# Costava/heightmap-ray-marcher

Measured on AMD Instinct MI355X. Metric: ray-steps/s at 3840x2160, 4096^2 heightmap, higher is better.
Workload: dtype f64; 1 GPU; C3: 4096x4096 heightmap, 3840x2160, spherical hfov 180, step_dist 0.25, grid_width 1; ray_steps_per_frame=1197030646, rays_per_frame=8294400, hits_per_frame=1006074, parallelism=1 GPU, launches back to back on one stream

## Files before the change

### heightmap-ray-marcher_amd/__init__.py

```python
from .lib import (
    Camera, Config, HmrmError, Scene, SceneParams, Stats,
    Ray, RayHit, TraceParams, SegmentParams, Sun, Water, CellMapParams, CellRect, GeometryPlanes, LightPlanes, MAP_TOWARDS_POINT, MAP_WEIGHT, MAP_DIFFUSE, MAP_NO_SHADOWS, RAY_END, TRACE_INTERIOR, SHADE_DIFFUSE, SHADE_NO_SHADOWS, RAY_DTYPE, RAY_HIT_DTYPE, RAY_MISS, RAY_HIT, RAY_CAPPED, MAX_RAYS, as_rays,
    PERSPECTIVE, SPHERICAL, ORTHOGRAPHIC, NEAREST, BILINEAR, NEAREST_F32,
    HMRM_OK, HMRM_E_ARG, HMRM_E_IO, HMRM_E_IMAGE, HMRM_E_CONFIG, HMRM_E_DEVICE, HMRM_E_NOTERM,
    EXPORTED_SYMBOLS, LIB_PATH, NO_PROBE, AA_FACTORS, aa_flags,
    band_local_rows, debug_frame, degrees_to_rads, device_count, image_load, image_load_memory, kernel_src_sha,
    last_error, mip_layout, level_state, calibrate, pick_kernel, plan_order, rcp_error, orbit_camera, orbit_frame_owner, png_encode, record_orbit, record_orbit_multi, record_orbit_shaded, record_orbit_baked, record_orbit_water, LIGHT_U8, LIGHT_U16, WATER_OWN_COLOR, WATER_BAKED, Haze, HAZE_SKY, HAZE_LINEAR, HAZE_EXP, HAZE_EXP2, MAX_HAZE_ENTRIES, haze_table, MAX_VIEWS, camera_array, views_tables, shade_flags, map_flags, sky_directions, render_multi, set_device, write_png, write_ppm, write_pfm,
)
from . import synth
```

### heightmap-ray-marcher_amd/csrc/api_aux.cpp

```cpp
#include <algorithm>
#include <cstdlib>
#include <cstring>
#include <fstream>
#include <new>
#include <sstream>

#include "api_internal.hpp"
#include "config.hpp"
#include "host_pool.hpp"
#include "image_io.hpp"

struct hmrm_config {
	hmrm::Config cfg;
	std::string log_cache, warn_cache;
};

extern "C" {

int hmrm_debug_kernel_choice(const hmrm_scene *s) {
	if (!s) return fail(HMRM_E_ARG, "NULL argument");
	std::lock_guard<std::mutex> lk(const_cast<hmrm_scene *>(s)->mu);
	if (s->knobs.kernel != 0) return s->knobs.kernel;
	return s->choice.use_group ? (s->choice.with_records ? 3 : 1) : 0;
}
// ... 335 lines not shown
	if (cam->projection == HMRM_SPHERICAL) {
		double *cc = tables, *cs = tables + W, *rs = tables + 2 * W, *rc2 = tables + 2 * W + H;
		const int nc = cam->width, nr = cam->height;
		hmrm::parallel_ranges(nc + nr, 1024, [&](int b, int e) {
			if (b < nc) hmrm::fill_col_tables(hc, b, std::min(e, nc), cc, cs);
			if (e > nc) hmrm::fill_row_tables(hc, std::max(b, nc) - nc, e - nc, rs, rc2);
		});
	}
	double *o = out25;
	for (int i = 0; i < 3; ++i) *o++ = f.cam[i];
	for (int i = 0; i < 3; ++i) *o++ = f.upper_left[i];
	for (int i = 0; i < 3; ++i) *o++ = f.plane_right[i];
	for (int i = 0; i < 3; ++i) *o++ = f.plane_down[i];
	for (int i = 0; i < 3; ++i) *o++ = f.look[i];
	for (int i = 0; i < 3; ++i) *o++ = f.c0[i];
	for (int i = 0; i < 3; ++i) *o++ = f.c1[i];
	*o++ = f.nudge;
	*o++ = f.step_dist;
	*o++ = (double)f.grid_pow2;
	*o++ = f.inv_grid_width;
	return HMRM_OK;
}

int hmrm_debug_pick_kernel(int32_t forced, int32_t use_other, int32_t records_ok, int32_t scene_verdict, int32_t scene_with_records,
                           int32_t *with_records_after) {
	hmrm::KernelChoice choice;
	choice.use_group = scene_verdict != 0;
	choice.probed = choice.use_group;
	choice.with_records = scene_with_records != 0;
	const int k = hmrm::pick_fast_kernel(forced, use_other != 0, records_ok != 0, choice);
	if (with_records_after) *with_records_after = choice.with_records ? 1 : 0;
	return k;
}

int hmrm_debug_level_state(int32_t level, int32_t young, int32_t min_level, int32_t out[8]) {
	if (!out || level < 0 || level > hmrm::kMipLevels || min_level < 0 || min_level >= hmrm::kMipLevels)
		return fail(HMRM_E_ARG, "hmrm_debug_level_state: bad argument");
	const uint32_t b = (uint32_t)(hmrm::level_state_table() >> (8 * level)) & 0xffu;
	const int hs = (int)(b & 31u), back = (int)(b >> 5);
	const int lstep = hmrm::level_step(young ? 0 : -1);
	out[0] = hs;
	out[1] = back;
	out[2] = (back + 1) << hs;
	out[3] = lstep;
	out[4] = hmrm::level_coarser(level, lstep);
	out[5] = hmrm::level_finer(level, lstep, min_level);
// ... 31 lines not shown
```

### heightmap-ray-marcher_amd/csrc/api_internal.hpp

```cpp
#pragma once
#include <hip/hip_runtime_api.h>

#include <cstddef>
#include <cstdint>
#include <mutex>
#include <string>
#include <vector>

#include "../../include/hmrm.h"
#include "frame.hpp"
#include "launch_order.hpp"
#include "render.hpp"

#pragma GCC visibility push(hidden)
namespace hmrm {
extern thread_local std::string g_error;
int fail(int code, const std::string &msg);
}
using namespace hmrm;

#define HIP_TRY(expr)                                                                         \
	do {                                                                                      \
		hipError_t e_ = (expr);                                                               \
		if (e_ != hipSuccess)                                                                 \
			return fail(HMRM_E_DEVICE, std::string(#expr) + ": " + hipGetErrorString(e_));    \
	} while (0)

struct Knobs {
	int64_t step_cap = (int64_t)1 << 26;
	int kernel = 0;
	bool tile_order = true;
	int order_mode = 2;
	int diag_mode = 0;
	int min_level = -1;
	int finest_pause = -1;
	bool order_verbose = false;
	bool try_group = true;
	int min_plane_shift = 0;
	int seg_n = 0;
	int seg_b[3] = {0, 0, 0}, seg_c[3] = {0, 0, 0};
};

template <bool kPinned> struct Scratch {
	void *ptr = nullptr;
	size_t cap = 0;
	int reserve(size_t bytes) {
		if (bytes <= cap) return HMRM_OK;
		release();
		if (kPinned) HIP_TRY(hipHostMalloc(&ptr, bytes, hipHostMallocDefault));
		else HIP_TRY(hipMalloc(&ptr, bytes));
		cap = bytes;
		return HMRM_OK;
	}
	template <class T> T *as() const { return static_cast<T *>(ptr); }
	void release() {
		if (ptr) (void)(kPinned ? hipHostFree(ptr) : hipFree(ptr));
		ptr = nullptr;
		cap = 0;
	}
// ... 217 lines not shown
```

### heightmap-ray-marcher_amd/csrc/api_launch.cpp

```cpp
#include <algorithm>
#include <cstdio>
#include <cstring>

#include "api_internal.hpp"
#include "host_pool.hpp"

static_assert(sizeof(hmrm_sun) == 48, "hmrm_sun has padding");
static_assert(sizeof(hmrm_camera) == 3 * sizeof(int32_t) + 4 + 8 * sizeof(double), "hmrm_camera has padding");
static_assert(sizeof(hmrm_scene_params) == 6 * sizeof(double), "hmrm_scene_params has padding");
static_assert(HMRM_SHADE_DIFFUSE == hmrm::kShadeDiffuse && HMRM_SHADE_NO_SHADOWS == hmrm::kShadeNoShadows, "route_frame's flag bits");

namespace {

int ensure_meas(StreamCtx *c) {
	if (!c->d_meas) HIP_TRY(hipMalloc((void **)&c->d_meas, (size_t)kMaxMeasRows * hmrm::kMeasureStride * sizeof(unsigned long long)));
	if (!c->h_meas) {
		const size_t n = (size_t)kFrameSlots * 2 * kMaxMeasRows * sizeof(unsigned long long);
		HIP_TRY(hipHostMalloc((void **)&c->h_meas, n, hipHostMallocMapped));
		HIP_TRY(hipHostGetDevicePointer((void **)&c->h_meas_dev, c->h_meas, 0));
	}
	return HMRM_OK;
}

bool others_idle(hmrm_scene *s, StreamCtx *c) {
// ... 192 lines not shown

int prepare_frame(hmrm_scene *s, StreamCtx *c, const hmrm_camera *cam, hmrm::DevFrame *f, FrameSlot **slot_out) {
	const uint64_t thr_bits = *(const uint64_t *)&s->thr_max;
	FrameSlot *slot = nullptr;
	for (FrameSlot &sl : c->slots)
		if (sl.valid && memcmp(&sl.cam, cam, sizeof *cam) == 0 && memcmp(&sl.params, &s->params, sizeof s->params) == 0 &&
		    sl.thr_max_bits == thr_bits)
			slot = &sl;
	if (!slot) {
		slot = &c->slots[0];
		for (FrameSlot &sl : c->slots)
			if (!sl.valid || sl.stamp < slot->stamp) {
				slot = &sl;
				if (!sl.valid) break;
			}
		slot->valid = false;
		if (slot->cal.in_flight >= 0) HIP_TRY(hipEventSynchronize(slot->measured));
		slot->cal.reset();
		hmrm::HostCamera hc;
		to_host_camera(cam, &hc);
		double *cc = nullptr, *cs = nullptr, *rs = nullptr, *rc = nullptr;
		const size_t W = (size_t)cam->width, H = (size_t)cam->height;
		if (cam->projection == HMRM_SPHERICAL) {
			const size_t n = 2 * W + 2 * H;
			if (n > c->arena_n) {
				HIP_TRY(hipStreamSynchronize(c->stream));
				if (c->d_arena) (void)hipFree(c->d_arena);
				if (c->h_arena) (void)hipHostFree(c->h_arena);
				c->d_arena = c->h_arena = nullptr;
				c->arena_n = 0;
				for (FrameSlot &sl : c->slots) {
					if (sl.cam.projection == HMRM_SPHERICAL) sl.valid = false;
					sl.d_tables = sl.h_tables = nullptr;
				}
				const size_t per = (n + 31) & ~(size_t)31;
				HIP_TRY(hipMalloc((void **)&c->d_arena, per * kFrameSlots * sizeof(double)));
				HIP_TRY(hipHostMalloc((void **)&c->h_arena, per * kFrameSlots * sizeof(double), hipHostMallocMapped));
				HIP_TRY(hipHostGetDevicePointer((void **)&c->h_arena_dev, c->h_arena, 0));
				c->arena_n = per;
			}
			const size_t idx = (size_t)(slot - c->slots);
			slot->d_tables = c->d_arena + idx * c->arena_n;
			slot->h_tables = c->h_arena + idx * c->arena_n;
			if (!slot->uploaded) HIP_TRY(hipEventCreateWithFlags(&slot->uploaded, hipEventDisableTiming));
			else HIP_TRY(hipEventSynchronize(slot->uploaded));
			cc = slot->h_tables;
			cs = cc + W;
// ... 3 lines not shown
		hmrm::DevFrame &fr = slot->frame;
		hmrm::build_frame(hc, s->map_w, s->map_h, s->params.min_height, s->params.max_height, s->params.grid_width,
		                  &fr, nullptr, nullptr, nullptr, nullptr);
		if (cam->projection == HMRM_SPHERICAL) {
			const FrameSlot *row_donor = nullptr, *col_donor = nullptr;
			for (const FrameSlot &o : c->slots) {
				if (!o.valid || &o == slot || o.cam.projection != HMRM_SPHERICAL || !o.h_tables) continue;
				if (o.cam.width != cam->width || o.cam.hfov != cam->hfov) continue;
				if (!col_donor && o.cam.hang == cam->hang) col_donor = &o;
				if (!row_donor && o.cam.height == cam->height && o.cam.vang == cam->vang) row_donor = &o;
			}
			if (col_donor) memcpy(cc, col_donor->h_tables, 2 * W * sizeof(double));
			if (row_donor) memcpy(rs, row_donor->h_tables + 2 * (size_t)row_donor->cam.width, 2 * H * sizeof(double));
			const int nc = col_donor ? 0 : cam->width, nr = row_donor ? 0 : cam->height;
			if (nc + nr > 0)
				hmrm::parallel_ranges(nc + nr, 1024, [&](int b, int e) {
					if (b < nc) hmrm::fill_col_tables(hc, b, std::min(e, nc), cc, cs);
					if (e > nc) hmrm::fill_row_tables(hc, std::max(b, nc) - nc, e - nc, rs, rc);
				});
		}
		slot->row_cost.assign(((size_t)cam->height + kCostRows - 1) / kCostRows, 0.0f);
		hmrm::estimate_row_costs(fr, cc, cs, rs, rc, kCostRows, slot->row_cost.data());
		if (cam->projection == HMRM_SPHERICAL) {
			HIP_TRY(hmrm::launch_upload_tables(c->h_arena_dev + (slot->h_tables - c->h_arena), slot->d_tables, 2 * W + 2 * H, c->stream));
			HIP_TRY(hipEventRecord(slot->uploaded, c->stream));
			fr.col_cos_ha = slot->d_tables;
			fr.col_sin_ha = slot->d_tables + W;
			fr.row_sin_va = slot->d_tables + 2 * W;
			fr.row_cos_va = slot->d_tables + 2 * W + H;
		}
		if (cam->sampling == HMRM_BILINEAR) {
			const int rc2 = ensure_bilinear_pyramid(s);
			if (rc2 != HMRM_OK) return rc2;
		}
		finish_frame_record(s, cam->sampling, &fr);
		slot->cam = *cam;
		slot->params = s->params;
		slot->thr_max_bits = thr_bits;
		slot->valid = true;
		for (size_t k = s->settled.size(); k-- > 0;) {
			const hmrm_scene::SettledOrder &so = s->settled[k];
			if (memcmp(&so.cam, cam, sizeof *cam) != 0 || memcmp(&so.params, &s->params, sizeof s->params) != 0 || so.thr_max_bits != thr_bits) continue;
			slot->cal.adopt(so.order);
			break;
		}
	}
	slot->stamp = ++s->clock;
	*f = slot->frame;
	apply_scene_knobs(s, f);
	if (slot_out) *slot_out = slot;
	return HMRM_OK;
}

void finish_frame_record(const hmrm_scene *s, int sampling, hmrm::DevFrame *fr) {
	fr->thr_max = sampling == HMRM_BILINEAR ? s->thr_max_bil : s->thr_max;
	fr->min_level = 0;
	while (fr->min_level < hmrm::kMipLevels - 1 && hmrm::win_cells(fr->min_level) < fr->min_window)
		++fr->min_level;
	fr->mipbuf = s->d_mipbuf;
	fr->mipbuf_bil = s->d_mipbuf_bil;
	fr->mip_row = s->mip_row;
	fr->mip_plane_shift = s->mip_plane_shift;
}

void apply_scene_knobs(const hmrm_scene *s, hmrm::DevFrame *f) {
	f->step_cap = s->knobs.step_cap;
	f->diag_mode = s->knobs.diag_mode;
	if (s->knobs.min_level >= 0) f->min_level = s->knobs.min_level;
	if (s->knobs.finest_pause >= 0) f->finest_pause = s->knobs.finest_pause;
}

int pick_views_kernel(hmrm_scene *s, StreamCtx *c, int sampling, ViewsKernel *out) {
	const bool huge_side = s->map_w >= (1 << 24) || s->map_h >= (1 << 24);
	const hmrm::FrameRoute route = hmrm::route_frame(s->knobs.kernel, huge_side, sampling, false, true, false, 0u);
	if (route.refused) return fail(HMRM_E_ARG, "maps with a side of 2^24 cells or more support nearest sampling only");
	int rc = wait_for_measure_fence(s, c);
	if (rc) return rc;
	poll_shadow_probe(s);
	const bool use_group = s->knobs.kernel == 0 && s->knobs.try_group && s->choice.use_group;
	out->literal = route.literal;
	out->kind = (hmrm::FastKernel)hmrm::pick_fast_kernel(s->knobs.kernel, use_group, sampling == 0 && s->d_records, s->choice);
	if (!route.literal && out->kind == hmrm::kRecords && (rc = ensure_records(s))) return rc;
	return HMRM_OK;
}

int acquire_view_stage(StreamCtx *c, size_t doubles, uint64_t stamp, ViewStage **out) {
	ViewStage *pick = nullptr, *oldest = &c->view_stages[0];
	for (ViewStage &v : c->view_stages) {
		if (v.stamp < oldest->stamp) oldest = &v;
		bool free_now = !v.used;
// ... 123 lines not shown
```

### heightmap-ray-marcher_amd/csrc/api_scene.cpp

```cpp
#include <cstdio>
#include <cstdlib>
#include <cstring>
#include <new>
#include <vector>

#include "api_internal.hpp"

namespace hmrm {

thread_local std::string g_error;

int fail(int code, const std::string &msg) {
	g_error = msg;
	return code;
}

int set_error(int code, const char *msg) { return fail(code, msg ? msg : ""); }

}

namespace {

Knobs read_knobs() {
	Knobs k;
	if (const char *s = getenv("HMRM_STEP_CAP")) {
		const long long v = atoll(s);
		if (v > 0) k.step_cap = v > 0x7fffffffLL ? 0x7fffffffLL : (int64_t)v;
	}
	if (const char *s = getenv("HMRM_KERNEL")) k.kernel = strcmp(s, "simple") == 0 ? 2 : (strcmp(s, "group") == 0 ? 1 : (strcmp(s, "rec") == 0 ? 3 : 0));
	if (const char *s = getenv("HMRM_TILE_ORDER")) {
		k.tile_order = s[0] != '0';
		if (s[0] == '1' || s[0] == '2') k.order_mode = s[0] - '0';
	}
	if (const char *s = getenv("HMRM_DIAG_ITERS")) k.diag_mode = atoi(s);
	if (const char *s = getenv("HMRM_ORDER_VERBOSE")) k.order_verbose = s[0] == '1';
	if (const char *s = getenv("HMRM_TRY_GROUP")) k.try_group = s[0] != '0';
	if (const char *s = getenv("HMRM_TILE_SEGMENTS")) {
		int b = 0, c = 0, used = 0;
		while (k.seg_n < 3 && sscanf(s, "%d:%d%n", &b, &c, &used) == 2 && b >= 0 && c > 0) {
			k.seg_b[k.seg_n] = b;
			k.seg_c[k.seg_n] = c;
			++k.seg_n;
			s += used;
			if (*s != ',') break;
			++s;
		}
	}
	if (const char *s = getenv("HMRM_DEBUG_PLANE_SHIFT")) {
		const int v = atoi(s);
		if (v > 0 && v <= 28) k.min_plane_shift = v;
	}
	if (const char *s = getenv("HMRM_MIN_LEVEL"))
		if (s[0] >= '0' && s[0] < '0' + hmrm::kMipLevels) k.min_level = s[0] - '0';
	if (const char *s = getenv("HMRM_FINEST_PAUSE"))
		if (s[0] >= '0' && s[0] <= '9') k.finest_pause = s[0] - '0';
	return k;
}

void destroy_ctx(StreamCtx *c) {
// ... 424 lines not shown
```

### heightmap-ray-marcher_amd/csrc/camera.cpp

```cpp
#include "frame.hpp"

#include <cmath>
#include <cstring>

namespace hmrm {
namespace {

struct Vec3 {
	double x, y, z;
};
inline Vec3 operator+(Vec3 a, Vec3 b) { return Vec3{a.x + b.x, a.y + b.y, a.z + b.z}; }
inline Vec3 operator-(Vec3 a, Vec3 b) { return Vec3{a.x - b.x, a.y - b.y, a.z - b.z}; }
inline Vec3 operator-(Vec3 a) { return Vec3{-a.x, -a.y, -a.z}; }
inline Vec3 operator*(double s, Vec3 v) { return Vec3{s * v.x, s * v.y, s * v.z}; }
inline Vec3 cross(Vec3 a, Vec3 b) {
	return Vec3{a.y * b.z - b.y * a.z, a.z * b.x - b.z * a.x, a.x * b.y - b.x * a.y};
}
inline double dot(Vec3 a, Vec3 b) {
	const double px = a.x * b.x, py = a.y * b.y, pz = a.z * b.z;
	return px + py + pz;
}
inline Vec3 normalize(Vec3 v) {
	const double inv = 1.0 / std::sqrt(dot(v, v));
	return Vec3{v.x * inv, v.y * inv, v.z * inv};
// ... 10 lines not shown
}

void fill_col_tables(const HostCamera &cam, int32_t begin, int32_t end, double *col_cos_ha, double *col_sin_ha) {
	const double hfov = cam.hfov;
	const double ul_hang = cam.hang + (hfov / 2.0);
	for (int32_t px = begin; px < end; ++px) {
		const double w = (double)px / (cam.width - 1);
		const double ha = ul_hang - w * hfov;
		col_cos_ha[px] = std::cos(ha);
		col_sin_ha[px] = std::sin(ha);
	}
}

void fill_row_tables(const HostCamera &cam, int32_t begin, int32_t end, double *row_sin_va, double *row_cos_va) {
	const double aspect = (double)cam.width / cam.height;
	const double vfov = cam.hfov / aspect;
	const double ul_vang = cam.vang - (vfov / 2.0);
	for (int32_t py = begin; py < end; ++py) {
		const double h = (double)py / (cam.height - 1);
		const double va = ul_vang + h * vfov;
		row_sin_va[py] = std::sin(va);
		row_cos_va[py] = std::cos(va);
	}
}

void fill_scene_fields(int32_t map_w, int32_t map_h, double min_height, double max_height, double grid_width,
                       double step_dist, DevFrame *f) {
	f->map_w = map_w;
	f->map_h = map_h;

	f->c0[0] = 0.0;
	f->c0[1] = 0.0;
	f->c0[2] = min_height;
	f->c1[0] = f->c0[0] + map_w * grid_width;
	f->c1[1] = f->c0[1] - map_h * grid_width;
	f->c1[2] = max_height;

	f->grid_width = grid_width;
	f->nudge = grid_width * 0.01;
	f->step_dist = step_dist;

	int e = 0;
	const double m = std::frexp(grid_width, &e);
	f->grid_pow2 = (std::isfinite(grid_width) && m == 0.5 && e > -1000 && e < 1000) ? 1 : 0;
	f->inv_grid_width = 1.0 / grid_width;
	f->grid_mode = grid_width == 1.0 ? 0 : (f->grid_pow2 ? 1 : 2);
// ... 74 lines not shown
```

### heightmap-ray-marcher_amd/csrc/frame.hpp

```cpp
#pragma once
#include <stdint.h>

namespace hmrm {

struct DevFrame {
	int32_t screen_w, screen_h;
	int32_t projection;
	int32_t map_w, map_h;
	uint8_t bg[4];
	double cam[3];
	double upper_left[3], plane_right[3], plane_down[3];
	double look[3];
	const double *col_cos_ha, *col_sin_ha;
	const double *row_sin_va, *row_cos_va;
	double c0[3], c1[3];
	double grid_width;
	double nudge;
	double step_dist;
	double inv_grid_width;
	int32_t grid_pow2;
	int32_t grid_mode;
	double thr_max;
	int64_t step_cap;
	const float *mipbuf;
// ... 93 lines not shown
	uint32_t spare1[2];
};
static_assert(sizeof(WindowRecord) == 32, "two 16-byte loads");
static_assert(kRecLevel >= kDenseFrom && kLevelStep == 1, "the record level's windows: 16 cells, every 4");
#if defined(__HIPCC__)
__host__ __device__
#endif
inline int rec_row(int map_w) { return (map_w + 3) >> 2; }

struct RowMap {
	int32_t row_begin;
	int32_t local_rows;
	int32_t band_rows;
	int32_t band_index, band_count;
	int32_t seg_first[3];
	int32_t seg_delta[4];
	unsigned long long *measure;
};
constexpr int kMeasureStride = 33;
constexpr int kOrderSegs = 4;

static_assert(sizeof(DevFrame) == 352,"DevFrame must not grow");

struct BatchRay { double pos[3], dir[3]; };
struct BatchHit {
	double point[3];
	double entry_d;
	uint32_t steps;
	int32_t cell_x, cell_y;
	uint8_t rgba[4];
	uint32_t status;
	uint32_t reserved;
};
static_assert(sizeof(BatchRay) == 48 && sizeof(BatchHit) == 56, "hmrm_ray / hmrm_ray_hit");
struct RayBatch {
	const BatchRay *rays;
	BatchHit *hits;
	int64_t n;
};
constexpr int kBatchW = 8;

struct SegRules {
	const uint32_t *max_steps;
	uint32_t limit;
	uint32_t interior;
};
// ... 61 lines not shown
	uint32_t flags;
};
constexpr uint32_t kHazeSky = 2u;
constexpr int kMaxHazeEntries = 4096;

struct HostCamera {
	int32_t width, height, projection;
	uint8_t bg_r, bg_g, bg_b, sampling;
	double hfov, hang, vang, pos[3], ortho_width, step_dist;
};

void build_frame(const HostCamera &cam, int32_t map_w, int32_t map_h,
                 double min_height, double max_height, double grid_width,
                 DevFrame *out,
                 double *col_cos_ha, double *col_sin_ha,
                 double *row_sin_va, double *row_cos_va);

void fill_scene_fields(int32_t map_w, int32_t map_h, double min_height, double max_height, double grid_width,
                       double step_dist, DevFrame *out);

void fill_col_tables(const HostCamera &cam, int32_t begin, int32_t end, double *col_cos_ha, double *col_sin_ha);
void fill_row_tables(const HostCamera &cam, int32_t begin, int32_t end, double *row_sin_va, double *row_cos_va);

void estimate_row_costs(const DevFrame &f, const double *col_cos_ha, const double *col_sin_ha,
                        const double *row_sin_va, const double *row_cos_va, int rows_per_sample, float *out);

}
```

### heightmap-ray-marcher_amd/csrc/march_frame.hpp

```cpp
#pragma once
#include "march.hpp"

namespace hmrm {

#ifdef HMRM_TIMELINE
__device__ __forceinline__ void timeline_wave_done(unsigned long long t0);
static void timeline_before_launch(dim3 grid, int tiles_y, const RowMap &rows);
#endif

template <int PROJ, bool STATS, int GWM, int LEAP, int SAMP, bool AA>
__global__ __launch_bounds__(kBlockThreads, HMRM_MIN_WAVES) HMRM_OCCUPANCY_ATTR void k_render_fast(const DevFrame f, const RowMap rows,
                                                     const double *__restrict__ thr,
                                                     const uint32_t *__restrict__ cmap,
                                                     uint32_t *__restrict__ out, int64_t out_stride_px,
                                                     int tiles_y, StatsOut st) {
#ifdef HMRM_TIMELINE
	const unsigned long long tl_t0 = __builtin_amdgcn_s_memrealtime();
#endif
	unsigned long long wave_t0 = 0;
	if (!STATS && rows.measure) wave_t0 = __builtin_amdgcn_s_memrealtime();
	const int tile_y = render_wave_tile<Family<FramesOf<STATS, AA>, PROJ, GWM, LEAP, SAMP>>(
	    f, rows, thr, cmap, out, out_stride_px, tiles_y, st, (int)blockIdx.x, blockIdx.z * 32768u + blockIdx.y, (int)(threadIdx.x >> 6),
	    (int)(threadIdx.x & 63));
	if (!STATS && rows.measure && tile_y >= 0 && (threadIdx.x & 63) == 0) {
		const unsigned long long took = __builtin_amdgcn_s_memrealtime() - wave_t0;
		unsigned long long *rec = rows.measure + (size_t)tile_y * kMeasureStride;
		if (blockIdx.x == 0 && threadIdx.x == 0) rec[0] = wave_t0;
		atomicMax(&rec[1 + (blockIdx.x & 31u)], took);
	}
#ifdef HMRM_TIMELINE
	if (!STATS) timeline_wave_done(tl_t0);
#endif
}

template <bool AA>
static hipError_t launch_fast(const DevFrame &f, const RowMap &rows, const double *d_thr_f64, const float *d_thr32,
                              const uint32_t *d_cmap, uint32_t *d_out, int64_t out_stride_px,
                              unsigned long long *d_counters, uint32_t *d_steps, double *d_entry, bool stats,
                              FastKernel kernel, const WindowRecord *d_records, hipStream_t stream) {
	DevFrame fr = f;
	const double *d_thr = nullptr;
	if (const hipError_t e = select_tables(&fr, kernel, d_thr_f64, d_thr32, d_records, &d_thr); e != hipSuccess) return e;
	const LaunchGrid g = tile_grid(f, rows);
	if (g.tiles_y == 0) return g.err;
	const StatsOut st{d_counters, d_steps, d_entry};
#ifdef HMRM_TIMELINE
	if (!stats) timeline_before_launch(g.grid, g.tiles_y, rows);
#endif
	auto launch = [&](auto instrumented) {
		dispatch_march(f.projection, f.grid_mode, kernel, f.sampling, [&](auto proj, auto gwm, auto leap, auto samp) {
			hipLaunchKernelGGL((k_render_fast<proj(), decltype(instrumented)::value, gwm(), leap(), samp(), AA>), g.grid,
			                   dim3(kBlockThreads), 0, stream, fr, rows, d_thr, d_cmap, d_out, out_stride_px, g.tiles_y, st);
		});
	};
	if (stats) launch(std::true_type{});
	else launch(std::false_type{});
	return hipGetLastError();
}

}
```

### heightmap-ray-marcher_amd/lib.py

```python
from __future__ import annotations

import ctypes as C
import os

import numpy as np

_HERE = os.path.dirname(os.path.abspath(__file__))
LIB_PATH = os.path.join(_HERE, "libhmrm.so")

HMRM_OK = 0
HMRM_E_ARG, HMRM_E_IO, HMRM_E_IMAGE, HMRM_E_CONFIG, HMRM_E_DEVICE, HMRM_E_NOTERM = -1, -2, -3, -4, -5, -6
PERSPECTIVE, SPHERICAL, ORTHOGRAPHIC = 1, 2, 3
NEAREST, BILINEAR, NEAREST_F32 = 0, 1, 2
_PROJ_NAMES = {"perspective": 1, "spherical": 2, "orthographic": 3}


NO_PROBE = 1
AA_FACTORS = (1, 2, 4, 8)


def aa_flags(n: int) -> int:
    return (int(n) & 15) << 8


# ... 296 lines not shown
        "hmrm_config_get_haze": (None, [vp, C.POINTER(Haze), vp]),
        "hmrm_config_haze_law": (i32, [vp]),
        "hmrm_config_haze_density": (C.c_double, [vp]),
        "hmrm_config_haze_far": (C.c_double, [vp]),
        "hmrm_render_shaded": (C.c_int, [vp, C.POINTER(Camera), C.POINTER(Sun), C.c_uint32, vp, C.c_size_t]),
        "hmrm_render_shaded_aa": (C.c_int, [vp, C.POINTER(Camera), C.POINTER(Sun), C.c_uint32, i32, vp, C.c_size_t]),
        "hmrm_render_shaded_begin": (C.c_int, [vp, C.POINTER(Camera), C.POINTER(Sun), C.c_uint32, C.c_uint32, C.POINTER(i32)]),
        "hmrm_render_shaded_device_begin": (C.c_int, [vp, C.POINTER(Camera), C.POINTER(Sun), C.c_uint32, vp, C.c_size_t, C.c_uint32,
                                                      C.POINTER(i32)]),
        "hmrm_scene_set_light": (C.c_int, [vp, vp, C.c_size_t, i32, C.c_uint32]),
        "hmrm_scene_set_light_device": (C.c_int, [vp, vp, C.c_size_t, i32, C.c_uint32, vp]),
        "hmrm_scene_bake_light": (C.c_int, [vp, C.POINTER(CellMapParams), dp, i32]),
        "hmrm_scene_clear_light": (C.c_int, [vp]),
        "hmrm_scene_light": (C.c_int, [vp, vp, C.c_size_t, C.POINTER(C.c_uint32)]),
        "hmrm_render_baked": (C.c_int, [vp, C.POINTER(Camera), C.c_uint32, i32, vp, C.c_size_t]),
        "hmrm_render_baked_begin": (C.c_int, [vp, C.POINTER(Camera), C.c_uint32, C.c_uint32, C.POINTER(i32)]),
        "hmrm_render_baked_device_begin": (C.c_int, [vp, C.POINTER(Camera), C.c_uint32, vp, C.c_size_t, C.c_uint32, C.POINTER(i32)]),
        "hmrm_record_orbit_baked": (C.c_int, [C.POINTER(vp), i32, C.POINTER(Camera), C.c_double, C.c_double, C.c_double,
                                              C.c_double, i32, C.c_char_p, C.c_longlong, i32, i32, C.c_uint32, C.c_uint32]),
        "hmrm_config_baked_light": (i32, [vp]),
        "hmrm_pick": (C.c_int, [vp, C.POINTER(Camera), i32, i32, C.POINTER(RayHit)]),
        "hmrm_debug_ray": (C.c_int, [vp, C.POINTER(Camera), i32, i32, dp, dp, dp]),
        "hmrm_debug_frame": (C.c_int, [C.POINTER(Camera), C.POINTER(SceneParams), i32, i32, vp, vp]),
        "hmrm_debug_plan_order": (C.c_int, [vp, i32, i32, C.POINTER(i32), C.POINTER(i32), vp]),
        "hmrm_debug_rcp_error": (C.c_int, [i32, C.c_uint64, C.c_uint64, i32, i32, dp, C.POINTER(C.c_uint64)]),
        "hmrm_last_kernel_ms": (C.c_double, []),
        "hmrm_bench_kernel_ms": (C.c_double, [vp, C.POINTER(Camera), i32]),
        "hmrm_orbit_camera": (None, [C.POINTER(Camera), C.c_double, C.c_double, C.c_double, C.c_double, i32, i32,
                                     C.POINTER(Camera)]),
        "hmrm_record_orbit": (C.c_int, [vp, C.POINTER(Camera), C.c_double, C.c_double, C.c_double, C.c_double, i32,
                                        C.c_char_p, C.c_longlong, i32, i32]),
        "hmrm_config_record_mode": (i32, [vp]),
        "hmrm_config_devices": (i32, [vp]),
        "hmrm_config_antialias": (i32, [vp]),
        "hmrm_config_interior": (i32, [vp]),
        "hmrm_config_shadows": (i32, [vp]),
        "hmrm_config_shading": (i32, [vp]),
        "hmrm_config_sky_light": (i32, [vp]),
        "hmrm_config_sun_scope": (i32, [vp]),
        "hmrm_config_sun_map_path": (C.c_char_p, [vp]),
        "hmrm_config_sun_map_lift": (C.c_double, [vp]),
        "hmrm_config_sky_map_path": (C.c_char_p, [vp]),
        "hmrm_config_sky_map_rings": (None, [vp, C.POINTER(i32), C.POINTER(i32)]),
        "hmrm_config_range_map_path": (C.c_char_p, [vp]),
        "hmrm_config_get_sun": (None, [vp, C.POINTER(Sun)]),
        "hmrm_record_orbit_multi": (C.c_int, [C.POINTER(vp), i32, C.POINTER(Camera), C.c_double, C.c_double, C.c_double,
# ... 86 lines not shown


def _check(rc: int, allow=()):
    if rc != HMRM_OK and rc not in allow:
        raise HmrmError(rc, last_error())
    return rc


def _ptr(a: np.ndarray):
    return a.ctypes.data_as(C.c_void_p)


def device_count() -> int:
    n = lib.hmrm_device_count()
    if n < 0:
        raise HmrmError(n, last_error())
    return n


def set_device(i: int):
    _check(lib.hmrm_set_device(int(i)))


_ENV_KNOBS = ("HMRM_KERNEL", "HMRM_STEP_CAP", "HMRM_TILE_ORDER", "HMRM_DIAG_ITERS", "HMRM_MIN_LEVEL", "HMRM_FINEST_PAUSE", "HMRM_TILE_SEGMENTS", "HMRM_ORDER_VERBOSE", "HMRM_TRY_GROUP")


def shade_flags(diffuse=True, shadows=True) -> int:
    return (SHADE_DIFFUSE if diffuse else 0) | (0 if shadows else SHADE_NO_SHADOWS)


def map_flags(point=False, weight=False, diffuse=False, shadows=True) -> int:
    return ((MAP_TOWARDS_POINT if point else 0) | (MAP_WEIGHT if weight else 0) | (MAP_DIFFUSE if diffuse else 0)
            | (0 if shadows else MAP_NO_SHADOWS))


def sky_directions(rings: int, per_ring: int) -> np.ndarray:
    n = int(rings) * int(per_ring)
    out = np.zeros((max(min(n, 256), 1), 3), dtype=np.float64)
    rc = lib.hmrm_sky_directions(int(rings), int(per_ring), out.ctypes.data_as(C.POINTER(C.c_double)))
    if rc < 0:
        raise HmrmError(rc, last_error())
    return out[:rc]


def _as_rect(rect):
    if rect is None or isinstance(rect, CellRect):
        return rect
# ... 457 lines not shown

    def bench_kernel_ms(self, cam: Camera, iters: int) -> float:
        self._sync_env()
        ms = lib.hmrm_bench_kernel_ms(self._h, C.byref(cam), int(iters))
        if ms < 0:
            raise HmrmError(HMRM_E_DEVICE, last_error())
        return ms


def debug_frame(cam: Camera, params: SceneParams, map_w: int, map_h: int):
    out = np.empty(25, dtype=np.float64)
    tables = np.empty(2 * cam.width + 2 * cam.height, dtype=np.float64)
    _check(lib.hmrm_debug_frame(C.byref(cam), C.byref(params), map_w, map_h, _ptr(out), _ptr(tables)))
    W, H = cam.width, cam.height
    rec = {"cam": out[0:3], "upper_left": out[3:6], "plane_right": out[6:9], "plane_down": out[9:12],
           "look": out[12:15], "c0": out[15:18], "c1": out[18:21], "nudge": out[21], "step_dist": out[22],
           "grid_pow2": int(out[23]), "inv_grid_width": out[24]}
    if cam.projection == SPHERICAL:
        rec.update(col_cos_ha=tables[0:W], col_sin_ha=tables[W:2 * W],
                   row_sin_va=tables[2 * W:2 * W + H], row_cos_va=tables[2 * W + H:])
    return rec


def mip_layout(map_w: int, map_h: int):
    row, shift, levels = C.c_int32(), C.c_int32(), C.c_int32()
    rc = lib.hmrm_debug_mip_layout(int(map_w), int(map_h), C.byref(row), C.byref(shift), C.byref(levels))
    if rc < 0:
        raise HmrmError(rc, last_error())
    return row.value, shift.value, levels.value, bool(rc)


def level_state(level: int, young: bool, min_level: int):
    out = (C.c_int32 * 8)()
    rc = lib.hmrm_debug_level_state(int(level), int(bool(young)), int(min_level), out)
    if rc < 0:
        raise HmrmError(rc, last_error())
    keys = ("stride_shift", "back", "cells", "lstep", "coarser", "finer", "at_finest", "byte")
    return dict(zip(keys, (int(v) for v in out))), int(rc)


def pick_kernel(forced=0, use_other=False, records_ok=True, verdict=False, verdict_with_records=False):
    after = C.c_int32()
    k = lib.hmrm_debug_pick_kernel(int(forced), int(use_other), int(records_ok), int(verdict), int(verdict_with_records), C.byref(after))
    return int(k), bool(after.value)


# ... 340 lines not shown
```

### include/hmrm.h

```cpp
#ifndef HMRM_H
#define HMRM_H

#include <stddef.h>
#include <stdint.h>

#ifdef __cplusplus
extern "C" {
#endif

#define HMRM_ABI_VERSION 1

enum {
	HMRM_OK          =  0,
	HMRM_E_ARG       = -1,
	HMRM_E_IO        = -2,
	HMRM_E_IMAGE     = -3,
	HMRM_E_CONFIG    = -4,
	HMRM_E_DEVICE    = -5,
	HMRM_E_NOTERM    = -6
};

enum {
	HMRM_PERSPECTIVE  = 1,
	HMRM_SPHERICAL    = 2,
// ... 269 lines not shown
	uint8_t  reserved[5];
} hmrm_haze;
int hmrm_render_haze(const hmrm_scene *scene, const hmrm_camera *cam, const hmrm_haze *haze, const uint8_t *table, int32_t factor,
                     uint8_t *rgba, size_t stride_bytes);
int hmrm_render_haze_device(const hmrm_scene *scene, const hmrm_camera *cam, const hmrm_haze *haze, const void *d_table,
                            int32_t factor, void *d_rgba, size_t stride_bytes, void *hip_stream);
int hmrm_haze_table(int32_t law, double density, int32_t n, uint8_t *out);

#define HMRM_MAX_VIEWS 65536
#define HMRM_MAX_VIEWS_STAGING (256u << 20)
int hmrm_render_views(const hmrm_scene *scene, const hmrm_camera *cams, int32_t n, uint32_t flags,
                      uint8_t *rgba, size_t stride_bytes, size_t view_stride_bytes);
int hmrm_render_views_device(const hmrm_scene *scene, const hmrm_camera *cams, int32_t n, uint32_t flags,
                             void *d_rgba, size_t stride_bytes, size_t view_stride_bytes, void *hip_stream);
int hmrm_debug_views_tables(const hmrm_camera *cams, int32_t n, int32_t *out_col_index, int32_t *out_row_index);

int hmrm_pick(const hmrm_scene *scene, const hmrm_camera *cam, int32_t px, int32_t py, hmrm_ray_hit *hit);

int hmrm_debug_ray(const hmrm_scene *scene, const hmrm_camera *cam,
                   int32_t px, int32_t py, double pos[3], double dir[3], double *entry_d);

int hmrm_debug_frame(const hmrm_camera *cam, const hmrm_scene_params *params,
                     int32_t map_w, int32_t map_h, double *out25, double *tables);

int hmrm_debug_plan_order(const uint64_t *records, int32_t tile_rows, int32_t rot, int32_t pieces_begin[3],
                          int32_t pieces_count[3], int32_t *tile_row_of_grid_row);

int hmrm_debug_calibrate(const uint64_t *records, int32_t launches, int32_t tile_rows, int32_t rot, int32_t may_probe,
                         int32_t scene_already_probed, const uint8_t *can_measure, int32_t *trial_used, int32_t *measured,
                         int32_t *group_kernel, int32_t *n_trials, int32_t *best, int32_t *scene_use_group,
                         int32_t *settled_at_launch);

int hmrm_debug_level_state(int32_t level, int32_t young, int32_t min_level, int32_t out[8]);

int hmrm_debug_rcp_error(int32_t mode, uint64_t count, uint64_t seed, int32_t exp_lo, int32_t exp_hi,
                         double *max_rel_err, uint64_t *hist64);

int hmrm_debug_mip_layout(int32_t map_w, int32_t map_h, int32_t *mip_row, int32_t *plane_shift, int32_t *levels);

int hmrm_debug_kernel_choice(const hmrm_scene *scene);

int hmrm_debug_read_records(const hmrm_scene *scene, void *records_out, double *thr_out);

int hmrm_debug_pick_kernel(int32_t forced, int32_t use_other, int32_t records_ok, int32_t scene_verdict, int32_t scene_with_records,
                           int32_t *with_records_after);

// ... 91 lines not shown
```

Before: 12540 billion ray-steps/s.

## Skip marching for 8x8 sky tiles proven to miss the heightmap box

On the host, per-row and per-column sign classes of the spherical ray directions are built, along with a per-row sky colour, and uploaded alongside the trig tables. In the fast kernel, a wave whose 8x8 tile is proven to point away from the heightmap bounding box writes the precomputed sky colour and skips the ray-march. This removes setup and marching cost for rays that can never hit terrain. It adds host table construction, a larger upload, a per-wave classification check, and an env knob to turn it off. It is gated off for stats, AA, and row maps not aligned to 8 rows.

```diff
diff --git a/heightmap-ray-marcher_amd/__init__.py b/heightmap-ray-marcher_amd/__init__.py
--- a/heightmap-ray-marcher_amd/__init__.py
+++ b/heightmap-ray-marcher_amd/__init__.py
@@ -4,7 +4,7 @@
     PERSPECTIVE, SPHERICAL, ORTHOGRAPHIC, NEAREST, BILINEAR, NEAREST_F32,
     HMRM_OK, HMRM_E_ARG, HMRM_E_IO, HMRM_E_IMAGE, HMRM_E_CONFIG, HMRM_E_DEVICE, HMRM_E_NOTERM,
     EXPORTED_SYMBOLS, LIB_PATH, NO_PROBE, AA_FACTORS, aa_flags,
-    band_local_rows, debug_frame, degrees_to_rads, device_count, image_load, image_load_memory, kernel_src_sha,
+    band_local_rows, debug_frame, debug_sky_tables, degrees_to_rads, device_count, image_load, image_load_memory, kernel_src_sha,
     last_error, mip_layout, level_state, calibrate, pick_kernel, plan_order, rcp_error, orbit_camera, orbit_frame_owner, png_encode, record_orbit, record_orbit_multi, record_orbit_shaded, record_orbit_baked, record_orbit_water, LIGHT_U8, LIGHT_U16, WATER_OWN_COLOR, WATER_BAKED, Haze, HAZE_SKY, HAZE_LINEAR, HAZE_EXP, HAZE_EXP2, MAX_HAZE_ENTRIES, haze_table, MAX_VIEWS, camera_array, views_tables, shade_flags, map_flags, sky_directions, render_multi, set_device, write_png, write_ppm, write_pfm,
 )
 from . import synth
diff --git a/heightmap-ray-marcher_amd/csrc/api_aux.cpp b/heightmap-ray-marcher_amd/csrc/api_aux.cpp
--- a/heightmap-ray-marcher_amd/csrc/api_aux.cpp
+++ b/heightmap-ray-marcher_amd/csrc/api_aux.cpp
@@ -381,6 +381,33 @@
 	return HMRM_OK;
 }
 
+int hmrm_debug_sky_tables(const hmrm_camera *cam, const hmrm_scene_params *params, int32_t map_w, int32_t map_h,
+                          uint32_t *row_miss_rgba, uint32_t *row_class, uint32_t *col_class, uint32_t box_side[3],
+                          int32_t box_side_known[3], uint8_t *proven) {
+	int rc = check_camera(cam);
+	if (rc) return rc;
+	if (!params || !row_miss_rgba || !row_class || !col_class) return fail(HMRM_E_ARG, "NULL argument");
+	if (cam->projection != HMRM_SPHERICAL) return fail(HMRM_E_ARG, "hmrm_debug_sky_tables: spherical cameras only");
+	hmrm::HostCamera hc;
+	to_host_camera(cam, &hc);
+	const size_t W = (size_t)cam->width, H = (size_t)cam->height;
+	std::vector<double> tables(2 * W + 2 * H);
+	double *cc = tables.data(), *cs = cc + W, *rs = cs + W, *rc2 = rs + H;
+	hmrm::DevFrame f;
+	hmrm::build_frame(hc, map_w, map_h, params->min_height, params->max_height, params->grid_width, &f, cc, cs, rs, rc2);
+	hmrm::build_sky_tables(f, cc, cs, rs, rc2, row_miss_rgba, row_class, col_class);
+	for (int i = 0; i < 3; ++i) {
+		if (box_side) box_side[i] = f.box_side[i];
+		if (box_side_known) box_side_known[i] = f.box_side_known[i];
+	}
+	if (proven) {
+		const int gx = hmrm::sky_groups(cam->width), gy = hmrm::sky_groups(cam->height);
+		for (int y = 0; y < gy; ++y)
+			for (int x = 0; x < gx; ++x) proven[(size_t)y * gx + x] = hmrm::sky_tile_proven(f, row_class[y], col_class[x]) ? 1 : 0;
+	}
+	return HMRM_OK;
+}
+
 int hmrm_debug_pick_kernel(int32_t forced, int32_t use_other, int32_t records_ok, int32_t scene_verdict, int32_t scene_with_records,
                            int32_t *with_records_after) {
 	hmrm::KernelChoice choice;
diff --git a/heightmap-ray-marcher_amd/csrc/api_internal.hpp b/heightmap-ray-marcher_amd/csrc/api_internal.hpp
--- a/heightmap-ray-marcher_amd/csrc/api_internal.hpp
+++ b/heightmap-ray-marcher_amd/csrc/api_internal.hpp
@@ -35,6 +35,7 @@
 	int min_level = -1;
 	int finest_pause = -1;
 	bool order_verbose = false;
+	bool sky_tiles = true;
 	bool try_group = true;
 	int min_plane_shift = 0;
 	int seg_n = 0;
diff --git a/heightmap-ray-marcher_amd/csrc/api_launch.cpp b/heightmap-ray-marcher_amd/csrc/api_launch.cpp
--- a/heightmap-ray-marcher_amd/csrc/api_launch.cpp
+++ b/heightmap-ray-marcher_amd/csrc/api_launch.cpp
@@ -238,7 +238,7 @@
 		double *cc = nullptr, *cs = nullptr, *rs = nullptr, *rc = nullptr;
 		const size_t W = (size_t)cam->width, H = (size_t)cam->height;
 		if (cam->projection == HMRM_SPHERICAL) {
-			const size_t n = 2 * W + 2 * H;
+			const size_t n = 2 * W + 2 * H + hmrm::sky_table_doubles(cam->width, cam->height);
 			if (n > c->arena_n) {
 				HIP_TRY(hipStreamSynchronize(c->stream));
 				if (c->d_arena) (void)hipFree(c->d_arena);
@@ -288,7 +288,12 @@
 		slot->row_cost.assign(((size_t)cam->height + kCostRows - 1) / kCostRows, 0.0f);
 		hmrm::estimate_row_costs(fr, cc, cs, rs, rc, kCostRows, slot->row_cost.data());
 		if (cam->projection == HMRM_SPHERICAL) {
-			HIP_TRY(hmrm::launch_upload_tables(c->h_arena_dev + (slot->h_tables - c->h_arena), slot->d_tables, 2 * W + 2 * H, c->stream));
+			const size_t sky_doubles = hmrm::sky_table_doubles(cam->width, cam->height);
+			uint32_t *sky = reinterpret_cast<uint32_t *>(rc + H);
+			sky[2 * sky_doubles - 1] = 0u;
+			hmrm::build_sky_tables(fr, cc, cs, rs, rc, sky, sky + H, sky + H + hmrm::sky_groups(cam->height));
+			fr.diag_mode = hmrm::kSkyTilesUsable;
+			HIP_TRY(hmrm::launch_upload_tables(c->h_arena_dev + (slot->h_tables - c->h_arena), slot->d_tables, 2 * W + 2 * H + sky_doubles, c->stream));
 			HIP_TRY(hipEventRecord(slot->uploaded, c->stream));
 			fr.col_cos_ha = slot->d_tables;
 			fr.col_sin_ha = slot->d_tables + W;
@@ -331,7 +336,7 @@
 
 void apply_scene_knobs(const hmrm_scene *s, hmrm::DevFrame *f) {
 	f->step_cap = s->knobs.step_cap;
-	f->diag_mode = s->knobs.diag_mode;
+	f->diag_mode = (s->knobs.diag_mode & ~hmrm::kSkyTilesUsable) | (s->knobs.sky_tiles ? (f->diag_mode & hmrm::kSkyTilesUsable) : 0);
 	if (s->knobs.min_level >= 0) f->min_level = s->knobs.min_level;
 	if (s->knobs.finest_pause >= 0) f->finest_pause = s->knobs.finest_pause;
 }
diff --git a/heightmap-ray-marcher_amd/csrc/api_scene.cpp b/heightmap-ray-marcher_amd/csrc/api_scene.cpp
--- a/heightmap-ray-marcher_amd/csrc/api_scene.cpp
+++ b/heightmap-ray-marcher_amd/csrc/api_scene.cpp
@@ -35,6 +35,7 @@
 	if (const char *s = getenv("HMRM_DIAG_ITERS")) k.diag_mode = atoi(s);
 	if (const char *s = getenv("HMRM_ORDER_VERBOSE")) k.order_verbose = s[0] == '1';
 	if (const char *s = getenv("HMRM_TRY_GROUP")) k.try_group = s[0] != '0';
+	if (const char *s = getenv("HMRM_SKY_TILES")) k.sky_tiles = s[0] != '0';
 	if (const char *s = getenv("HMRM_TILE_SEGMENTS")) {
 		int b = 0, c = 0, used = 0;
 		while (k.seg_n < 3 && sscanf(s, "%d:%d%n", &b, &c, &used) == 2 && b >= 0 && c > 0) {
diff --git a/heightmap-ray-marcher_amd/csrc/camera.cpp b/heightmap-ray-marcher_amd/csrc/camera.cpp
--- a/heightmap-ray-marcher_amd/csrc/camera.cpp
+++ b/heightmap-ray-marcher_amd/csrc/camera.cpp
@@ -56,6 +56,43 @@
 		row_sin_va[py] = std::sin(va);
 		row_cos_va[py] = std::cos(va);
 	}
+}
+
+void build_sky_tables(const DevFrame &f, const double *col_cos_ha, const double *col_sin_ha, const double *row_sin_va,
+                      const double *row_cos_va, uint32_t *row_miss_rgba, uint32_t *row_class, uint32_t *col_class) {
+	auto high = [](double v) {
+		uint64_t b;
+		memcpy(&b, &v, sizeof b);
+		return (uint32_t)(b >> 32);
+	};
+	auto sign_class = [&](double v, uint32_t pos, uint32_t neg) -> uint32_t {
+		const uint32_t h = high(v);
+		if ((((h >> 20) & 0x7ffu) - 823u) >= 201u) return 0u;
+		return (h >> 31) ? neg : pos;
+	};
+	auto channel = [](double v) { return (uint32_t)(v < 255.0 ? v : 255.0); };
+	const int32_t W = f.screen_w, H = f.screen_h;
+	for (int32_t g = 0; g < sky_groups(H); ++g) row_class[g] = kSkyRowZAway | kSkyRowSinPos | kSkyRowSinNeg;
+	for (int32_t g = 0; g < sky_groups(W); ++g) col_class[g] = kSkyColCosPos | kSkyColCosNeg | kSkyColSinPos | kSkyColSinNeg;
+	for (int32_t py = 0; py < H; ++py) {
+		const double dz = row_cos_va[py];
+		uint32_t r = f.bg[0], g = f.bg[1], b = f.bg[2];
+		if (dz > 0.0) {
+			const double zz = dz * dz;
+			const double r_ = 220.0 * zz + (double)f.bg[0];
+			const double g_ = 240.0 * zz + (double)f.bg[1];
+			const double b_ = 255.0 * dz + (double)f.bg[2];
+			r = channel(r_);
+			g = channel(g_);
+			b = channel(b_);
+		}
+		row_miss_rgba[py] = r | (g << 8) | (b << 16) | 0xff000000u;
+		const uint32_t hd = high(dz);
+		const bool z_away = f.box_side_known[2] != 0 && (((hd >> 20) & 0x7ffu) - 523u) < 1000u && ((f.box_side[2] ^ hd) >> 31) != 0u;
+		row_class[py / kSkyGroup] &= (z_away ? kSkyRowZAway : 0u) | sign_class(row_sin_va[py], kSkyRowSinPos, kSkyRowSinNeg);
+	}
+	for (int32_t px = 0; px < W; ++px)
+		col_class[px / kSkyGroup] &= sign_class(col_cos_ha[px], kSkyColCosPos, kSkyColCosNeg) | sign_class(col_sin_ha[px], kSkyColSinPos, kSkyColSinNeg);
 }
 
 void fill_scene_fields(int32_t map_w, int32_t map_h, double min_height, double max_height, double grid_width,
diff --git a/heightmap-ray-marcher_amd/csrc/frame.hpp b/heightmap-ray-marcher_amd/csrc/frame.hpp
--- a/heightmap-ray-marcher_amd/csrc/frame.hpp
+++ b/heightmap-ray-marcher_amd/csrc/frame.hpp
@@ -1,4 +1,5 @@
 #pragma once
+#include <stddef.h>
 #include <stdint.h>
 
 namespace hmrm {
@@ -139,6 +140,27 @@
 
 static_assert(sizeof(DevFrame) == 352,"DevFrame must not grow");
 
+constexpr int32_t kSkyTilesUsable = 0x40000000;
+constexpr int kSkyGroup = 8;
+constexpr uint32_t kSkyRowZAway = 1u, kSkyRowSinPos = 2u, kSkyRowSinNeg = 4u;
+constexpr uint32_t kSkyColCosPos = 1u, kSkyColCosNeg = 2u, kSkyColSinPos = 4u, kSkyColSinNeg = 8u;
+inline int sky_groups(int32_t n) { return (n + kSkyGroup - 1) / kSkyGroup; }
+inline size_t sky_table_words(int32_t w, int32_t h) { return (size_t)h + (size_t)sky_groups(h) + (size_t)sky_groups(w); }
+inline size_t sky_table_doubles(int32_t w, int32_t h) { return (sky_table_words(w, h) + 1) / 2; }
+#if defined(__HIPCC__)
+__host__ __device__
+#endif
+inline bool sky_tile_proven(const DevFrame &f, uint32_t row_class, uint32_t col_class) {
+	const uint32_t rs = (row_class >> 1) & 3u;
+	const uint32_t cx = col_class & 3u, cy = (col_class >> 2) & 3u;
+	return (row_class & kSkyRowZAway) != 0u ||
+	       (f.box_side_known[0] != 0 && rs != 0u && cx != 0u && ((rs ^ cx) >> 1) != (f.box_side[0] >> 31)) ||
+	       (f.box_side_known[1] != 0 && rs != 0u && cy != 0u && ((rs ^ cy) >> 1) != (f.box_side[1] >> 31));
+}
+inline bool sky_rows_aligned(const RowMap &rows) {
+	return rows.band_rows > 0 ? rows.band_rows % kSkyGroup == 0 : rows.row_begin % kSkyGroup == 0;
+}
+
 struct BatchRay { double pos[3], dir[3]; };
 struct BatchHit {
 	double point[3];
@@ -246,6 +268,9 @@
 void fill_col_tables(const HostCamera &cam, int32_t begin, int32_t end, double *col_cos_ha, double *col_sin_ha);
 void fill_row_tables(const HostCamera &cam, int32_t begin, int32_t end, double *row_sin_va, double *row_cos_va);
 
+void build_sky_tables(const DevFrame &f, const double *col_cos_ha, const double *col_sin_ha, const double *row_sin_va,
+                      const double *row_cos_va, uint32_t *row_miss_rgba, uint32_t *row_class, uint32_t *col_class);
+
 void estimate_row_costs(const DevFrame &f, const double *col_cos_ha, const double *col_sin_ha,
                         const double *row_sin_va, const double *row_cos_va, int rows_per_sample, float *out);
 
diff --git a/heightmap-ray-marcher_amd/csrc/march_frame.hpp b/heightmap-ray-marcher_amd/csrc/march_frame.hpp
--- a/heightmap-ray-marcher_amd/csrc/march_frame.hpp
+++ b/heightmap-ray-marcher_amd/csrc/march_frame.hpp
@@ -7,6 +7,26 @@
 __device__ __forceinline__ void timeline_wave_done(unsigned long long t0);
 static void timeline_before_launch(dim3 grid, int tiles_y, const RowMap &rows);
 #endif
+
+__device__ __forceinline__ bool sky_tile_done(const DevFrame &f, const RowMap &rows, uint32_t *__restrict__ out, int64_t out_stride_px,
+                                              int tiles_y, int *tile_y) {
+	static_assert(kWaveW == kSkyGroup && kWaveH == kSkyGroup, "a wave's pixels lie in one row group and one column group");
+	if ((f.diag_mode & kSkyTilesUsable) == 0) return false;
+	const int wave = __builtin_amdgcn_readfirstlane((int)(threadIdx.x >> 6));
+	const PixelId p0 = pixel_of_tile_lane(f, rows, tiles_y, (int)blockIdx.x, blockIdx.z * 32768u + blockIdx.y, wave, 0);
+	if (!p0.live) return false;
+	const uint32_t *__restrict__ row_miss_rgba = reinterpret_cast<const uint32_t *>(f.row_cos_va + f.screen_h);
+	typedef const uint32_t __attribute__((address_space(4))) *ConstWords;
+	const ConstWords row_class = (ConstWords)(uintptr_t)(row_miss_rgba + f.screen_h);
+	const ConstWords col_class = row_class + (uint32_t)(f.screen_h + kSkyGroup - 1) / (uint32_t)kSkyGroup;
+	if (!sky_tile_proven(f, row_class[(uint32_t)p0.py / (uint32_t)kSkyGroup], col_class[(uint32_t)p0.px / (uint32_t)kSkyGroup])) return false;
+	const int lane = (int)(threadIdx.x & 63);
+	const int px = p0.px + lane % kWaveW, dy = lane / kWaveW;
+	if (px < f.screen_w && p0.lrow + dy < rows.local_rows && p0.py + dy < f.screen_h)
+		out[(uint64_t)(uint32_t)(p0.lrow + dy) * (uint32_t)out_stride_px + (uint32_t)px] = row_miss_rgba[p0.py + dy];
+	*tile_y = p0.tile_y;
+	return true;
+}
 
 template <int PROJ, bool STATS, int GWM, int LEAP, int SAMP, bool AA>
 __global__ __launch_bounds__(kBlockThreads, HMRM_MIN_WAVES) HMRM_OCCUPANCY_ATTR void k_render_fast(const DevFrame f, const RowMap rows,
@@ -19,7 +39,11 @@
 #endif
 	unsigned long long wave_t0 = 0;
 	if (!STATS && rows.measure) wave_t0 = __builtin_amdgcn_s_memrealtime();
-	const int tile_y = render_wave_tile<Family<FramesOf<STATS, AA>, PROJ, GWM, LEAP, SAMP>>(
+	int tile_y = -1;
+	bool done = false;
+	if constexpr (PROJ == 2 && !STATS && !AA) done = sky_tile_done(f, rows, out, out_stride_px, tiles_y, &tile_y);
+	if (!done)
+	tile_y = render_wave_tile<Family<FramesOf<STATS, AA>, PROJ, GWM, LEAP, SAMP>>(
 	    f, rows, thr, cmap, out, out_stride_px, tiles_y, st, (int)blockIdx.x, blockIdx.z * 32768u + blockIdx.y, (int)(threadIdx.x >> 6),
 	    (int)(threadIdx.x & 63));
 	if (!STATS && rows.measure && tile_y >= 0 && (threadIdx.x & 63) == 0) {
@@ -39,6 +63,7 @@
                               unsigned long long *d_counters, uint32_t *d_steps, double *d_entry, bool stats,
                               FastKernel kernel, const WindowRecord *d_records, hipStream_t stream) {
 	DevFrame fr = f;
+	if (stats || AA || !sky_rows_aligned(rows)) fr.diag_mode &= ~kSkyTilesUsable;
 	const double *d_thr = nullptr;
 	if (const hipError_t e = select_tables(&fr, kernel, d_thr_f64, d_thr32, d_records, &d_thr); e != hipSuccess) return e;
 	const LaunchGrid g = tile_grid(f, rows);
diff --git a/heightmap-ray-marcher_amd/lib.py b/heightmap-ray-marcher_amd/lib.py
--- a/heightmap-ray-marcher_amd/lib.py
+++ b/heightmap-ray-marcher_amd/lib.py
@@ -342,6 +342,7 @@
         "hmrm_pick": (C.c_int, [vp, C.POINTER(Camera), i32, i32, C.POINTER(RayHit)]),
         "hmrm_debug_ray": (C.c_int, [vp, C.POINTER(Camera), i32, i32, dp, dp, dp]),
         "hmrm_debug_frame": (C.c_int, [C.POINTER(Camera), C.POINTER(SceneParams), i32, i32, vp, vp]),
+        "hmrm_debug_sky_tables": (C.c_int, [C.POINTER(Camera), C.POINTER(SceneParams), i32, i32, vp, vp, vp, vp, vp, vp]),
         "hmrm_debug_plan_order": (C.c_int, [vp, i32, i32, C.POINTER(i32), C.POINTER(i32), vp]),
         "hmrm_debug_rcp_error": (C.c_int, [i32, C.c_uint64, C.c_uint64, i32, i32, dp, C.POINTER(C.c_uint64)]),
         "hmrm_last_kernel_ms": (C.c_double, []),
@@ -474,7 +475,7 @@
     _check(lib.hmrm_set_device(int(i)))
 
 
-_ENV_KNOBS = ("HMRM_KERNEL", "HMRM_STEP_CAP", "HMRM_TILE_ORDER", "HMRM_DIAG_ITERS", "HMRM_MIN_LEVEL", "HMRM_FINEST_PAUSE", "HMRM_TILE_SEGMENTS", "HMRM_ORDER_VERBOSE", "HMRM_TRY_GROUP")
+_ENV_KNOBS = ("HMRM_KERNEL", "HMRM_STEP_CAP", "HMRM_TILE_ORDER", "HMRM_DIAG_ITERS", "HMRM_MIN_LEVEL", "HMRM_FINEST_PAUSE", "HMRM_TILE_SEGMENTS", "HMRM_ORDER_VERBOSE", "HMRM_TRY_GROUP", "HMRM_SKY_TILES")
 
 
 def shade_flags(diffuse=True, shadows=True) -> int:
@@ -978,6 +979,19 @@
     return rec
 
 
+def debug_sky_tables(cam: Camera, params: SceneParams, map_w: int, map_h: int):
+    W, H = cam.width, cam.height
+    gx, gy = (W + 7) // 8, (H + 7) // 8
+    rec = {"row_miss_rgba": np.zeros(H, dtype=np.uint32), "row_class": np.zeros(gy, dtype=np.uint32),
+           "col_class": np.zeros(gx, dtype=np.uint32), "box_side": np.zeros(3, dtype=np.uint32),
+           "box_side_known": np.zeros(3, dtype=np.int32)}
+    proven = np.zeros((gy, gx), dtype=np.uint8)
+    _check(lib.hmrm_debug_sky_tables(C.byref(cam), C.byref(params), map_w, map_h, _ptr(rec["row_miss_rgba"]), _ptr(rec["row_class"]),
+                                     _ptr(rec["col_class"]), _ptr(rec["box_side"]), _ptr(rec["box_side_known"]), _ptr(proven)))
+    rec["proven"] = proven.astype(bool)
+    return rec
+
+
 def mip_layout(map_w: int, map_h: int):
     row, shift, levels = C.c_int32(), C.c_int32(), C.c_int32()
     rc = lib.hmrm_debug_mip_layout(int(map_w), int(map_h), C.byref(row), C.byref(shift), C.byref(levels))
diff --git a/include/hmrm.h b/include/hmrm.h
--- a/include/hmrm.h
+++ b/include/hmrm.h
@@ -315,6 +315,10 @@
 
 int hmrm_debug_frame(const hmrm_camera *cam, const hmrm_scene_params *params,
                      int32_t map_w, int32_t map_h, double *out25, double *tables);
+
+int hmrm_debug_sky_tables(const hmrm_camera *cam, const hmrm_scene_params *params, int32_t map_w, int32_t map_h,
+                          uint32_t *row_miss_rgba, uint32_t *row_class, uint32_t *col_class, uint32_t box_side[3],
+                          int32_t box_side_known[3], uint8_t *proven);
 
 int hmrm_debug_plan_order(const uint64_t *records, int32_t tile_rows, int32_t rot, int32_t pieces_begin[3],
                           int32_t pieces_count[3], int32_t *tile_row_of_grid_row);
```

New measurement: 12590 billion ray-steps/s, median of 6. Within noise of the previous version (+0.4%).
